# speedinghzl/CCNet

Hardware: NVIDIA H100
Metric: cca_fwd_bwd_pixels_per_s (higher is better)
Workload: dtype f32

## Files before the change

ccnet_b200/csrc/cca_items.cuh:

```cuda
#pragma once

#ifndef __CUDACC__
#define CCA_HD inline
#else
#define CCA_HD __host__ __device__ __forceinline__
#endif

namespace cca {
namespace tc {

constexpr int kMaxTile = 112;
constexpr int kMaxNT = 8;

struct DirGeom {
    int L;
    int NL;
    int nt;
    int tl;
};

struct ItemSpace {
    int B, H, W;
    DirGeom col, row;
    int seg0, seg1, seg2;
    int per_sample, total;
    int nparts;
};

struct Item {
    int col;
    int b, line, iq, ik;
    int q0, lq, k0, lk;
    int j;
};

CCA_HD int tiles_for(int L) { return (L + kMaxTile - 1) / kMaxTile; }

CCA_HD DirGeom make_dir(int L, int NL)
{
    DirGeom g;
    g.L = L; g.NL = NL;
    g.nt = tiles_for(L);
    g.tl = (L + g.nt - 1) / g.nt;
    return g;
}

CCA_HD ItemSpace make_space(int B, int H, int W)
{
    ItemSpace s;
    s.B = B; s.H = H; s.W = W;
    s.col = make_dir(H, W);
    s.row = make_dir(W, H);
    s.seg0 = s.col.NL * s.col.nt;
    s.seg1 = s.col.NL * s.col.nt * (s.col.nt - 1);
    s.seg2 = s.row.NL * s.row.nt * s.row.nt;
    s.per_sample = s.seg0 + s.seg1 + s.seg2;
    s.total = B * s.per_sample;
    s.nparts = s.row.nt + s.col.nt;
    return s;
}

CCA_HD int max_tile(const ItemSpace &s) { return s.col.tl > s.row.tl ? s.col.tl : s.row.tl; }

CCA_HD Item decode_item(const ItemSpace &s, int idx)
{
    Item it;
    it.b = idx / s.per_sample;
    int j = idx - it.b * s.per_sample;
    it.j = j;
    const DirGeom *g;
    if (j < s.seg0) {
        it.col = 1; g = &s.col;
        it.line = j / g->nt; it.iq = j - it.line * g->nt; it.ik = 0;
    } else if (j < s.seg0 + s.seg1) {
        it.col = 1; g = &s.col;
        j -= s.seg0;
        const int per = g->nt - 1;
        const int li = j / per;
        it.ik = 1 + (j - li * per);
        it.line = li / g->nt; it.iq = li - it.line * g->nt;
    } else {
        it.col = 0; g = &s.row;
        j -= s.seg0 + s.seg1;
        const int li = j / g->nt;
        it.ik = j - li * g->nt;
        it.line = li / g->nt; it.iq = li - it.line * g->nt;
    }
    it.q0 = it.iq * g->tl; it.k0 = it.ik * g->tl;
    it.lq = g->L - it.q0 < g->tl ? g->L - it.q0 : g->tl;
    it.lk = g->L - it.k0 < g->tl ? g->L - it.k0 : g->tl;
    return it;
}

CCA_HD Item decode_item_in_sample(const ItemSpace &s, int b, int j) { return decode_item(s, b * s.per_sample + j); }

CCA_HD Item decode_item_lagged(const ItemSpace &s, int idx)
{
    const int np = s.seg0, nc = s.per_sample - s.seg0;
    if (idx < np) return decode_item_in_sample(s, 0, idx);
    const int x = idx - np;
    const int grp = x / s.per_sample, rem = x - grp * s.per_sample;
    if (grp < s.B - 1) {
        if (rem < np) return decode_item_in_sample(s, grp + 1, rem);
        return decode_item_in_sample(s, grp, np + (rem - np));
    }
    (void)nc;
    return decode_item_in_sample(s, s.B - 1, np + rem);
}
CCA_HD Item decode_item_order(const ItemSpace &s, int idx, int lag) { return lag ? decode_item_lagged(s, idx) : decode_item(s, idx); }
CCA_HD bool is_producer(const Item &it) { return it.col && it.ik == 0; }

CCA_HD long item_pixel(const ItemSpace &s, const Item &it, int r)
{
    return it.col ? ((long)it.b * s.H + (it.q0 + r)) * s.W + it.line : ((long)it.b * s.H + it.line) * s.W + (it.q0 + r);
}
CCA_HD int part_index(const ItemSpace &s, const Item &it) { return it.col ? s.row.nt + it.ik : it.ik; }
CCA_HD int qtile_part_index(const ItemSpace &s, const Item &it) { return it.col ? s.row.nt + it.iq : it.iq; }

CCA_HD long zero_share_bytes(long sample_bytes, int per_sample)
{
    const long s = (sample_bytes + per_sample - 1) / per_sample;
    return (s + 127) / 128 * 128;
}

}
}
```

ccnet_b200/csrc/cca_sm90.cuh:

```cuda
#pragma once
#include <cuda.h>
#include <cuda_runtime.h>
#include <stdint.h>

namespace sm90 {

__device__ __forceinline__ uint32_t smem_u32(const void *p) { return (uint32_t)__cvta_generic_to_shared(p); }

__device__ __forceinline__ void mbar_init(uint64_t *bar, uint32_t count)
{
    asm volatile("mbarrier.init.shared::cta.b64 [%0], %1;" ::"r"(smem_u32(bar)), "r"(count));
}
__device__ __forceinline__ void fence_mbar_init() { asm volatile("fence.mbarrier_init.release.cluster;" ::: "memory"); }
__device__ __forceinline__ void mbar_expect_tx(uint64_t *bar, uint32_t bytes)
{
    asm volatile("mbarrier.arrive.expect_tx.shared::cta.b64 _, [%0], %1;" ::"r"(smem_u32(bar)), "r"(bytes) : "memory");
}
__device__ __forceinline__ void mbar_arrive(uint64_t *bar)
{
    asm volatile("mbarrier.arrive.shared::cta.b64 _, [%0];" ::"r"(smem_u32(bar)) : "memory");
}
__device__ __forceinline__ bool mbar_try_wait(uint64_t *bar, uint32_t parity)
{
    uint32_t ok;
    asm volatile(
        "{\n\t.reg .pred p;\n\t"
        "mbarrier.try_wait.parity.shared::cta.b64 p, [%1], %2;\n\t"
        "selp.u32 %0, 1, 0, p;\n\t}"
        : "=r"(ok) : "r"(smem_u32(bar)), "r"(parity) : "memory");
    return ok != 0;
}
#ifndef CCA_SPIN_TRAP
#define CCA_SPIN_TRAP 0
#endif
__device__ __forceinline__ void mbar_wait(uint64_t *bar, uint32_t parity)
{
#if CCA_SPIN_TRAP
    uint32_t spins = 0;
    while (!mbar_try_wait(bar, parity)) {
        if (++spins > (1u << 26)) { __trap(); }
    }
#else
    while (!mbar_try_wait(bar, parity)) {}
#endif
}
__device__ __forceinline__ void wait_count(const unsigned int *cnt, unsigned int need)
{
    unsigned int v;
#if CCA_SPIN_TRAP
    unsigned int spins = 0;
#endif
    for (;;) {
        asm volatile("ld.acquire.gpu.global.u32 %0, [%1];" : "=r"(v) : "l"(cnt) : "memory");
        if (v >= need) return;
        __nanosleep(64);
#if CCA_SPIN_TRAP
        if (++spins > (1u << 24)) __trap();
#endif
    }
}
__device__ __forceinline__ void pdl_launch_dependents() { asm volatile("griddepcontrol.launch_dependents;" ::: "memory"); }
__device__ __forceinline__ void pdl_wait() { asm volatile("griddepcontrol.wait;" ::: "memory"); }

template <int N> __device__ __forceinline__ void setmaxnreg_dec() { asm volatile("setmaxnreg.dec.sync.aligned.u32 %0;" ::"n"(N)); }
template <int N> __device__ __forceinline__ void setmaxnreg_inc() { asm volatile("setmaxnreg.inc.sync.aligned.u32 %0;" ::"n"(N)); }

__device__ __forceinline__ void fence_proxy_async() { asm volatile("fence.proxy.async.shared::cta;" ::: "memory"); }

__device__ __forceinline__ void prefetch_tmap(const CUtensorMap *m)
{
    asm volatile("prefetch.tensormap [%0];" ::"l"(reinterpret_cast<uint64_t>(m)) : "memory");
}
__device__ __forceinline__ void tma_load_4d(void *dst, const CUtensorMap *m, uint64_t *bar, int c0, int c1, int c2, int c3)
{
    asm volatile(
        "cp.async.bulk.tensor.4d.shared::cluster.global.mbarrier::complete_tx::bytes [%0], [%1, {%3, %4, %5, %6}], [%2];"
        ::"r"(smem_u32(dst)), "l"(reinterpret_cast<uint64_t>(m)), "r"(smem_u32(bar)), "r"(c0), "r"(c1), "r"(c2), "r"(c3)
        : "memory");
}
__device__ __forceinline__ uint64_t l2_policy_evict_first()
{
    uint64_t pol;
    asm volatile("createpolicy.fractional.L2::evict_first.b64 %0, 1.0;" : "=l"(pol));
    return pol;
}
__device__ __forceinline__ uint64_t l2_policy_evict_last()
{
    uint64_t pol;
    asm volatile("createpolicy.fractional.L2::evict_last.b64 %0, 1.0;" : "=l"(pol));
    return pol;
}
__device__ __forceinline__ void tma_load_4d(void *dst, const CUtensorMap *m, uint64_t *bar, int c0, int c1, int c2, int c3, uint64_t pol)
{
    asm volatile(
        "cp.async.bulk.tensor.4d.shared::cluster.global.mbarrier::complete_tx::bytes.L2::cache_hint [%0], [%1, {%3, %4, %5, %6}], [%2], %7;"
        ::"r"(smem_u32(dst)), "l"(reinterpret_cast<uint64_t>(m)), "r"(smem_u32(bar)), "r"(c0), "r"(c1), "r"(c2), "r"(c3), "l"(pol)
        : "memory");
}
__device__ __forceinline__ void tma_store_4d(const CUtensorMap *m, const void *src, int c0, int c1, int c2, int c3)
{
    asm volatile("cp.async.bulk.tensor.4d.global.shared::cta.bulk_group [%0, {%2, %3, %4, %5}], [%1];"
                 ::"l"(reinterpret_cast<uint64_t>(m)), "r"(smem_u32(src)), "r"(c0), "r"(c1), "r"(c2), "r"(c3) : "memory");
}
__device__ __forceinline__ void tma_store_4d(const CUtensorMap *m, const void *src, int c0, int c1, int c2, int c3, uint64_t pol)
{
    asm volatile("cp.async.bulk.tensor.4d.global.shared::cta.bulk_group.L2::cache_hint [%0, {%2, %3, %4, %5}], [%1], %6;"
                 ::"l"(reinterpret_cast<uint64_t>(m)), "r"(smem_u32(src)), "r"(c0), "r"(c1), "r"(c2), "r"(c3), "l"(pol) : "memory");
}
__device__ __forceinline__ void tma_reduce_add_4d(const CUtensorMap *m, const void *src, int c0, int c1, int c2, int c3)
{
    asm volatile("cp.reduce.async.bulk.tensor.4d.global.shared::cta.add.tile.bulk_group [%0, {%2, %3, %4, %5}], [%1];"
                 ::"l"(reinterpret_cast<uint64_t>(m)), "r"(smem_u32(src)), "r"(c0), "r"(c1), "r"(c2), "r"(c3) : "memory");
}
__device__ __forceinline__ void tma_reduce_add_4d(const CUtensorMap *m, const void *src, int c0, int c1, int c2, int c3, uint64_t pol)
{
    asm volatile("cp.reduce.async.bulk.tensor.4d.global.shared::cta.add.tile.bulk_group.L2::cache_hint [%0, {%2, %3, %4, %5}], [%1], %6;"
                 ::"l"(reinterpret_cast<uint64_t>(m)), "r"(smem_u32(src)), "r"(c0), "r"(c1), "r"(c2), "r"(c3), "l"(pol) : "memory");
}
__device__ __forceinline__ void bulk_commit() { asm volatile("cp.async.bulk.commit_group;" ::: "memory"); }
template <int N> __device__ __forceinline__ void bulk_wait() { asm volatile("cp.async.bulk.wait_group %0;" ::"n"(N) : "memory"); }
template <int N> __device__ __forceinline__ void bulk_wait_read() { asm volatile("cp.async.bulk.wait_group.read %0;" ::"n"(N) : "memory"); }
__device__ __forceinline__ void fence_proxy_async_global() { asm volatile("fence.proxy.async.global;" ::: "memory"); }
__device__ __forceinline__ void publish_count(unsigned int *cnt)
{
    fence_proxy_async_global();
    __threadfence();
    atomicAdd(cnt, 1u);
}

constexpr uint32_t kSw128 = 1;
__device__ __forceinline__ uint64_t smem_desc(uint32_t smem_addr, uint32_t lbo_bytes, uint32_t sbo_bytes, uint32_t layout_type = 0)
{
    uint64_t d = 0;
    d |= (uint64_t)((smem_addr >> 4) & 0x3FFF);
    d |= (uint64_t)((lbo_bytes >> 4) & 0x3FFF) << 16;
    d |= (uint64_t)((sbo_bytes >> 4) & 0x3FFF) << 32;
    d |= (uint64_t)(layout_type & 3) << 62;
    return d;
}
__device__ __forceinline__ void wg_fence() { asm volatile("wgmma.fence.sync.aligned;" ::: "memory"); }
__device__ __forceinline__ void wg_commit() { asm volatile("wgmma.commit_group.sync.aligned;" ::: "memory"); }
template <int N> __device__ __forceinline__ void wg_wait() { asm volatile("wgmma.wait_group.sync.aligned %0;" ::"n"(N) : "memory"); }
template <int R> __device__ __forceinline__ void wg_acc_fence(float *d)
{
#pragma unroll
    for (int i = 0; i < R; ++i) asm volatile("" : "+f"(d[i])::"memory");
}

#define CCA_WGMMA_SS_N64(AB, TA, TB) asm volatile("{\n.reg .pred p;\nsetp.ne.b32 p, %34, 0;\n" \
    "wgmma.mma_async.sync.aligned.m64n64k16.f32." AB " {%0, %1, %2, %3, %4, %5, %6, %7, %8, %9, %10, %11, %12, %13, %14, %15, %16, %17, %18, %19, %20, %21, %22, %23, %24, %25, %26, %27, %28, %29, %30, %31}, %32, %33, p, 1, 1, " #TA ", " #TB ";\n}" \
    : "+f"(d[0]), "+f"(d[1]), "+f"(d[2]), "+f"(d[3]), "+f"(d[4]), "+f"(d[5]), "+f"(d[6]), "+f"(d[7]), "+f"(d[8]), "+f"(d[9]), "+f"(d[10]), "+f"(d[11]), "+f"(d[12]), "+f"(d[13]), "+f"(d[14]), "+f"(d[15]), "+f"(d[16]), "+f"(d[17]), "+f"(d[18]), "+f"(d[19]), "+f"(d[20]), "+f"(d[21]), "+f"(d[22]), "+f"(d[23]), "+f"(d[24]), "+f"(d[25]), "+f"(d[26]), "+f"(d[27]), "+f"(d[28]), "+f"(d[29]), "+f"(d[30]), "+f"(d[31]) : "l"(a), "l"(b), "r"(scale_d))
#define CCA_WGMMA_SS_N80(AB, TA, TB) asm volatile("{\n.reg .pred p;\nsetp.ne.b32 p, %42, 0;\n" \
    "wgmma.mma_async.sync.aligned.m64n80k16.f32." AB " {%0, %1, %2, %3, %4, %5, %6, %7, %8, %9, %10, %11, %12, %13, %14, %15, %16, %17, %18, %19, %20, %21, %22, %23, %24, %25, %26, %27, %28, %29, %30, %31, %32, %33, %34, %35, %36, %37, %38, %39}, %40, %41, p, 1, 1, " #TA ", " #TB ";\n}" \
    : "+f"(d[0]), "+f"(d[1]), "+f"(d[2]), "+f"(d[3]), "+f"(d[4]), "+f"(d[5]), "+f"(d[6]), "+f"(d[7]), "+f"(d[8]), "+f"(d[9]), "+f"(d[10]), "+f"(d[11]), "+f"(d[12]), "+f"(d[13]), "+f"(d[14]), "+f"(d[15]), "+f"(d[16]), "+f"(d[17]), "+f"(d[18]), "+f"(d[19]), "+f"(d[20]), "+f"(d[21]), "+f"(d[22]), "+f"(d[23]), "+f"(d[24]), "+f"(d[25]), "+f"(d[26]), "+f"(d[27]), "+f"(d[28]), "+f"(d[29]), "+f"(d[30]), "+f"(d[31]), "+f"(d[32]), "+f"(d[33]), "+f"(d[34]), "+f"(d[35]), "+f"(d[36]), "+f"(d[37]), "+f"(d[38]), "+f"(d[39]) : "l"(a), "l"(b), "r"(scale_d))
#define CCA_WGMMA_SS_N112(AB, TA, TB) asm volatile("{\n.reg .pred p;\nsetp.ne.b32 p, %58, 0;\n" \
    "wgmma.mma_async.sync.aligned.m64n112k16.f32." AB " {%0, %1, %2, %3, %4, %5, %6, %7, %8, %9, %10, %11, %12, %13, %14, %15, %16, %17, %18, %19, %20, %21, %22, %23, %24, %25, %26, %27, %28, %29, %30, %31, %32, %33, %34, %35, %36, %37, %38, %39, %40, %41, %42, %43, %44, %45, %46, %47, %48, %49, %50, %51, %52, %53, %54, %55}, %56, %57, p, 1, 1, " #TA ", " #TB ";\n}" \
    : "+f"(d[0]), "+f"(d[1]), "+f"(d[2]), "+f"(d[3]), "+f"(d[4]), "+f"(d[5]), "+f"(d[6]), "+f"(d[7]), "+f"(d[8]), "+f"(d[9]), "+f"(d[10]), "+f"(d[11]), "+f"(d[12]), "+f"(d[13]), "+f"(d[14]), "+f"(d[15]), "+f"(d[16]), "+f"(d[17]), "+f"(d[18]), "+f"(d[19]), "+f"(d[20]), "+f"(d[21]), "+f"(d[22]), "+f"(d[23]), "+f"(d[24]), "+f"(d[25]), "+f"(d[26]), "+f"(d[27]), "+f"(d[28]), "+f"(d[29]), "+f"(d[30]), "+f"(d[31]), "+f"(d[32]), "+f"(d[33]), "+f"(d[34]), "+f"(d[35]), "+f"(d[36]), "+f"(d[37]), "+f"(d[38]), "+f"(d[39]), "+f"(d[40]), "+f"(d[41]), "+f"(d[42]), "+f"(d[43]), "+f"(d[44]), "+f"(d[45]), "+f"(d[46]), "+f"(d[47]), "+f"(d[48]), "+f"(d[49]), "+f"(d[50]), "+f"(d[51]), "+f"(d[52]), "+f"(d[53]), "+f"(d[54]), "+f"(d[55]) : "l"(a), "l"(b), "r"(scale_d))
#define CCA_WGMMA_SS_T(OP, AB) \
    if (ta == 0 && tb == 0) OP(AB, 0, 0); \
    else if (ta == 0) OP(AB, 0, 1); \
    else if (tb == 0) OP(AB, 1, 0); \
    else OP(AB, 1, 1)
template <bool F16 = false> __device__ __forceinline__ void wgmma_ss_n64(float *d, uint64_t a, uint64_t b, int scale_d, int ta, int tb)
{
    if constexpr (F16) { CCA_WGMMA_SS_T(CCA_WGMMA_SS_N64, "f16.f16"); }
    else { CCA_WGMMA_SS_T(CCA_WGMMA_SS_N64, "bf16.bf16"); }
}
template <int TA, int TB> __device__ __forceinline__ void wgmma_ss_n32(float *d, uint64_t a, uint64_t b, int scale_d)
{
    asm volatile("{\n.reg .pred p;\nsetp.ne.b32 p, %18, 0;\n"
        "wgmma.mma_async.sync.aligned.m64n32k16.f32.bf16.bf16 {%0, %1, %2, %3, %4, %5, %6, %7, %8, %9, %10, %11, %12, %13, %14, %15}, %16, %17, p, 1, 1, %19, %20;\n}"
        : "+f"(d[0]), "+f"(d[1]), "+f"(d[2]), "+f"(d[3]), "+f"(d[4]), "+f"(d[5]), "+f"(d[6]), "+f"(d[7]), "+f"(d[8]), "+f"(d[9]), "+f"(d[10]), "+f"(d[11]), "+f"(d[12]), "+f"(d[13]), "+f"(d[14]), "+f"(d[15]) : "l"(a), "l"(b), "r"(scale_d), "n"(TA), "n"(TB));
}
template <bool F16 = false> __device__ __forceinline__ void wgmma_ss_n80(float *d, uint64_t a, uint64_t b, int scale_d, int ta, int tb)
{
    if constexpr (F16) { CCA_WGMMA_SS_T(CCA_WGMMA_SS_N80, "f16.f16"); }
    else { CCA_WGMMA_SS_T(CCA_WGMMA_SS_N80, "bf16.bf16"); }
}
template <bool F16 = false> __device__ __forceinline__ void wgmma_ss_n112(float *d, uint64_t a, uint64_t b, int scale_d, int ta, int tb)
{
    if constexpr (F16) { CCA_WGMMA_SS_T(CCA_WGMMA_SS_N112, "f16.f16"); }
    else { CCA_WGMMA_SS_T(CCA_WGMMA_SS_N112, "bf16.bf16"); }
}
#define CCA_WGMMA_RS_N64(AB) asm volatile("{\n.reg .pred p;\nsetp.ne.b32 p, %37, 0;\n" \
    "wgmma.mma_async.sync.aligned.m64n64k16.f32." AB " {%0, %1, %2, %3, %4, %5, %6, %7, %8, %9, %10, %11, %12, %13, %14, %15, %16, %17, %18, %19, %20, %21, %22, %23, %24, %25, %26, %27, %28, %29, %30, %31}, {%32, %33, %34, %35}, %36, p, 1, 1, 1;\n}" \
    : "+f"(d[0]), "+f"(d[1]), "+f"(d[2]), "+f"(d[3]), "+f"(d[4]), "+f"(d[5]), "+f"(d[6]), "+f"(d[7]), "+f"(d[8]), "+f"(d[9]), "+f"(d[10]), "+f"(d[11]), "+f"(d[12]), "+f"(d[13]), "+f"(d[14]), "+f"(d[15]), "+f"(d[16]), "+f"(d[17]), "+f"(d[18]), "+f"(d[19]), "+f"(d[20]), "+f"(d[21]), "+f"(d[22]), "+f"(d[23]), "+f"(d[24]), "+f"(d[25]), "+f"(d[26]), "+f"(d[27]), "+f"(d[28]), "+f"(d[29]), "+f"(d[30]), "+f"(d[31]) : "r"(a[0]), "r"(a[1]), "r"(a[2]), "r"(a[3]), "l"(b), "r"(scale_d))
template <bool F16 = false> __device__ __forceinline__ void wgmma_rs_n64_tb(float *d, const uint32_t *a, uint64_t b, int scale_d)
{
    if constexpr (F16) CCA_WGMMA_RS_N64("f16.f16");
    else CCA_WGMMA_RS_N64("bf16.bf16");
}

template <int N, bool F16 = false> __device__ __forceinline__ void wgmma_ss(float *d, uint64_t a, uint64_t b, int scale_d, int ta, int tb)
{
    static_assert(N == 64 || N == 80 || N == 112, "wgmma width");
    if constexpr (N == 64) wgmma_ss_n64<F16>(d, a, b, scale_d, ta, tb);
    else if constexpr (N == 80) wgmma_ss_n80<F16>(d, a, b, scale_d, ta, tb);
    else wgmma_ss_n112<F16>(d, a, b, scale_d, ta, tb);
}

}
```

ccnet_b200/csrc/cca_tc_bwd.cuh:

```cuda
#pragma once
#include "cca_items.cuh"
#include "cca_tc_common.cuh"

namespace cca {
namespace tc {

template <int LK, typename E, bool PL = false>
cudaError_t launch_bwd(const void *dout, const void *q, const void *k, const void *v, const void *out, const float *lse, float *delta,
                       unsigned int *counters, void *dq, void *dk, void *dv, Dims d, int delta_mode, cudaStream_t st,
                       const char **why);

struct BwdParams {
    ItemSpace sp;
    int C, Cq;
    long npix;
    const float *lse;
    float *delta;
    unsigned int *ddone;
    int delta_mode;
    int out_mode;
    unsigned int *cdone;
    int lag;
    int hints;
};

template <int LK, typename E> struct BwdSmem {
    using T = Tiles<LK, E>;
    static constexpr int kCh = T::H16 ? kNC : kNC / 2;
    static constexpr int kRSlot = T::kTile;
    static constexpr int off_qk = 0;
    static constexpr int off_p = off_qk + 2 * T::kSlot;
    static constexpr int off_ld = (off_p + T::kP + (16 - LK / 8) * T::kPlane + 1023) / 1024 * 1024;
    static constexpr int kTail = (128 - LK) * 128 + 256;
    static constexpr int kDsum = 1024;
    static constexpr int kBudget = 232448;
    static constexpr int kNLd = (kBudget - off_ld - kTail - kDsum) / (kRSlot + 16);
    static constexpr int off_tail = off_ld + kNLd * kRSlot;
    static constexpr int off_dsum = off_tail + kTail;
    static constexpr int off_bar = off_dsum + kDsum;
    static constexpr int kBytes = off_bar + 8 * 2 * kNLd;
    static_assert(kNLd >= 8, "ring depth: chunk n - 1's dO (staged dV) up to chunk n + 1's O");
    static_assert(off_p % 1024 == 0 && T::kP >= T::kSlot, "dK staging in the P / dS planes");
    static_assert(kBytes <= kBudget, "shared memory budget");
};

__device__ __forceinline__ bool calc_delta(const BwdParams &p, const Item &it) { return p.delta_mode == 0 || (it.col && it.ik == 0); }

template <int LK, typename E, bool PL = false>
__global__ void __launch_bounds__(kThreads, 1)
cca_tc_bwd_kernel(const __grid_constant__ CUtensorMap mqc, const __grid_constant__ CUtensorMap mqr,
                  const __grid_constant__ CUtensorMap mkc, const __grid_constant__ CUtensorMap mkr,
                  const __grid_constant__ CUtensorMap mvc, const __grid_constant__ CUtensorMap mvr,
                  const __grid_constant__ CUtensorMap mdoc, const __grid_constant__ CUtensorMap mdor,
                  const __grid_constant__ CUtensorMap moc, const __grid_constant__ CUtensorMap mor,
                  const __grid_constant__ CUtensorMap mdqc, const __grid_constant__ CUtensorMap mdqr,
                  const __grid_constant__ CUtensorMap mdkc, const __grid_constant__ CUtensorMap mdkr,
                  const __grid_constant__ CUtensorMap mdvc, const __grid_constant__ CUtensorMap mdvr, BwdParams p)
{
    using T = Tiles<LK, E>;
    using S = BwdSmem<LK, E>;
    constexpr bool H16 = kH16<E>, F16 = kF16<E>;
    constexpr int TERMS = H16 ? 1 : 3;
    constexpr int kNLd = S::kNLd;
    constexpr int kCh = S::kCh;
    constexpr int KP = LK / 16;
    constexpr int kQKBoxes = H16 ? 1 : 2;
    constexpr uint32_t LOP = T::kPP * T::kPlane;
    extern __shared__ __align__(1024) uint8_t smem[];
    uint64_t *bars = reinterpret_cast<uint64_t *>(smem + S::off_bar);
    uint64_t *full = bars, *empty = bars + kNLd;
    float *dsum = reinterpret_cast<float *>(smem + S::off_dsum);
    const int tid = threadIdx.x, warp = tid >> 5, lane = tid & 31;
    const int NCH = p.C / kCh;
    const int KQ = p.Cq / 16;
    const int nk = p.sp.total > (int)blockIdx.x ? (p.sp.total - (int)blockIdx.x + (int)gridDim.x - 1) / (int)gridDim.x : 0;
    auto item_of = [&](int k) { return decode_item_order(p.sp, (int)blockIdx.x + k * (int)gridDim.x, p.lag); };

    if (tid == 0) {
        for (int i = 0; i < kNLd; ++i) { mbar_init(&full[i], 1); mbar_init(&empty[i], 1); }
        fence_mbar_init();
        prefetch_tmap(&mqc); prefetch_tmap(&mqr); prefetch_tmap(&mkc); prefetch_tmap(&mkr); prefetch_tmap(&mvc); prefetch_tmap(&mvr);
        prefetch_tmap(&mdoc); prefetch_tmap(&mdor); prefetch_tmap(&moc); prefetch_tmap(&mor);
        prefetch_tmap(&mdqc); prefetch_tmap(&mdqr); prefetch_tmap(&mdkc); prefetch_tmap(&mdkr); prefetch_tmap(&mdvc); prefetch_tmap(&mdvr);
    }
    __syncthreads();

    if (tid < 128) {
        setmaxnreg_dec<kProducerRegs>();
        if (warp == 0 && lane == 0) {
            const uint64_t pol_keep = l2_policy_evict_last(), pol_stream = l2_policy_evict_first();
            uint32_t g = 0;
            auto ring = [&](const CUtensorMap *m, int c0, const Item &it, int start, bool last_use) {
                const int slot = g % kNLd;
                mbar_wait(&empty[slot], ((g / kNLd) & 1) ^ 1);
                mbar_expect_tx(&full[slot], S::kRSlot);
                uint8_t *dst = smem + S::off_ld + slot * S::kRSlot;
                const int cw = it.col ? it.line : start, ch = it.col ? start : it.line;
                if (p.hints == 1) {
                    const uint64_t pol = (is_producer(it) && !last_use) ? pol_keep : pol_stream;
                    tma_load_4d(dst, m, &full[slot], c0, cw, ch, it.b, pol);
                } else {
                    tma_load_4d(dst, m, &full[slot], c0, cw, ch, it.b);
                }
                ++g;
            };
            for (int k = 0; k < nk; ++k) {
                const Item it = item_of(k);
                const bool calc = calc_delta(p, it);
                for (int bx = 0; bx < kQKBoxes; ++bx) ring(it.col ? &mqc : &mqr, 32 * bx, it, it.q0, false);
                for (int bx = 0; bx < kQKBoxes; ++bx) ring(it.col ? &mkc : &mkr, 32 * bx, it, it.k0, false);
                for (int n = 0; n < NCH; ++n) {
                    ring(it.col ? &mvc : &mvr, n * kCh, it, it.k0, false);
                    ring(it.col ? &mdoc : &mdor, n * kCh, it, it.q0, false);
                    if (calc) ring(it.col ? &moc : &mor, n * kCh, it, it.q0, p.delta_mode == 1);
                }
            }
        }
    } else {
        setmaxnreg_inc<kConsumerRegs>();
        const int t = tid - 128, wg = t >> 7, wq = (t >> 5) & 3;
        const int rbase = 64 * wg + 16 * wq + (lane >> 2);
        const int cq = 2 * (lane & 3);
        const uint32_t qb = smem_u32(smem + S::off_qk), kb = qb + T::kSlot, ld_base = smem_u32(smem + S::off_ld);
        const uint32_t pb = smem_u32(smem + S::off_p);
        uint8_t *pgen = smem + S::off_p;
        const uint64_t pol_keep = l2_policy_evict_last(), pol_stream = l2_policy_evict_first();
        auto stage = [&](const float *acc, int nc, uint8_t *tile) {
#pragma unroll
            for (int h = 0; h < 2; ++h) {
                const int r = rbase + 8 * h;
                if (r >= LK) continue;
                uint8_t *row = tile + r * 128;
#pragma unroll
                for (int j = 0; j < 8; ++j) {
                    if (8 * j >= nc) break;
                    const int c = 8 * j + cq;
                    const int bx = H16 ? 0 : c >> 5, byte = H16 ? 2 * c : 4 * (c & 31);
                    uint8_t *dst = row + bx * T::kTile + ((((byte >> 4) ^ r) & 7) << 4) + (byte & 15);
                    if constexpr (H16) *reinterpret_cast<uint32_t *>(dst) = pack2<F16>(acc[4 * j + 2 * h], acc[4 * j + 2 * h + 1]);
                    else *reinterpret_cast<float2 *>(dst) = make_float2(acc[4 * j + 2 * h], acc[4 * j + 2 * h + 1]);
                }
            }
        };
        auto put = [&](const CUtensorMap *m, const uint8_t *tile, int boxes, int c0, int px0, const Item &it, bool prod, int part) {
            const int cw = it.col ? it.line : px0, ch = it.col ? px0 : it.line;
            const int ob = PL ? part * p.sp.B + it.b : it.b;
            for (int bx = 0; bx < boxes; ++bx) {
                const uint8_t *src = tile + bx * T::kTile;
                if (p.hints == 1) {
                    if (prod) tma_store_4d(m, src, c0 + 32 * bx, cw, ch, ob, pol_keep);
                    else tma_reduce_add_4d(m, src, c0 + 32 * bx, cw, ch, ob, pol_stream);
                } else {
                    if (prod) tma_store_4d(m, src, c0 + 32 * bx, cw, ch, ob);
                    else tma_reduce_add_4d(m, src, c0 + 32 * bx, cw, ch, ob);
                }
            }
            bulk_commit();
        };
        const int qboxes = H16 ? 1 : (p.Cq > 32 ? 2 : 1);
        pdl_wait();
        uint32_t g = 0;
        int pending = -1;
        int unpublished = -1;
        for (int k = 0; k < nk; ++k) {
            const Item it = item_of(k);
            const bool calc = calc_delta(p, it);
            const bool prod = PL || (p.out_mode == 1 && is_producer(it));
            long qpix[2];
            bool qok[2];
            float nlse[2];
            int self[2];
#pragma unroll
            for (int h = 0; h < 2; ++h) {
                const int r = rbase + 8 * h;
                qok[h] = r < it.lq;
                qpix[h] = item_pixel(p.sp, it, qok[h] ? r : 0);
                nlse[h] = qok[h] ? -p.lse[qpix[h]] * kLog2e : 0.f;
                self[h] = it.col ? it.q0 + r - it.k0 : -1;
            }
            {
                const uint8_t *src[2 * kQKBoxes];
#pragma unroll
                for (int i = 0; i < 2 * kQKBoxes; ++i) {
                    const uint32_t gi = g + i;
                    mbar_wait(&full[gi % kNLd], (gi / kNLd) & 1);
                    src[i] = smem + S::off_ld + (gi % kNLd) * S::kRSlot;
                }
                if constexpr (H16) {
                    constexpr int kV = T::kTile / 16, kPer = (kV + kConsumers - 1) / kConsumers;
                    uint4 v[2][kPer];
#pragma unroll
                    for (int i = 0; i < 2; ++i)
#pragma unroll
                        for (int j = 0; j < kPer; ++j)
                            if (t + kConsumers * j < kV) v[i][j] = reinterpret_cast<const uint4 *>(src[i])[t + kConsumers * j];
                    consumers_sync();
#pragma unroll
                    for (int i = 0; i < 2; ++i)
#pragma unroll
                        for (int j = 0; j < kPer; ++j)
                            if (t + kConsumers * j < kV) reinterpret_cast<uint4 *>(smem + S::off_qk + i * T::kSlot)[t + kConsumers * j] = v[i][j];
                    fence_proxy_async();
                    consumers_sync();
                } else {
                    convert_slot<LK, E, 4>(smem + S::off_qk, t, nullptr, src);
                }
                if (t == 0)
                    for (int i = 0; i < 2 * kQKBoxes; ++i) mbar_arrive(&empty[(g + i) % kNLd]);
                g += 2 * kQKBoxes;
            }
            {
                float acc[LK / 2];
                wg_fence();
                for (int ks = 0; ks < KQ; ++ks) {
                    wgmma_ss<LK, F16>(acc, desc_kmaj<LK, E>(qb, 64 * wg, ks, false), desc_kmaj<LK, E>(kb, 0, ks, false), ks > 0, 0, 0);
                    if constexpr (TERMS == 3) {
                        wgmma_ss<LK, F16>(acc, desc_kmaj<LK, E>(qb, 64 * wg, ks, false), desc_kmaj<LK, E>(kb, 0, ks, true), 1, 0, 0);
                        wgmma_ss<LK, F16>(acc, desc_kmaj<LK, E>(qb, 64 * wg, ks, true), desc_kmaj<LK, E>(kb, 0, ks, false), 1, 0, 0);
                    }
                }
                wg_commit();
                wg_wait<0>();
                wg_acc_fence<LK / 2>(acc);
                if (t == 0) {
                    if (unpublished >= 0) {
                        bulk_wait<0>();
                        publish_count(p.cdone + unpublished);
                        unpublished = -1;
                    } else {
                        bulk_wait_read<0>();
                    }
                }
                consumers_sync();
#pragma unroll
                for (int j = 0; j < LK / 8; ++j)
#pragma unroll
                    for (int h = 0; h < 2; ++h) {
                        const int r = rbase + 8 * h, c = 8 * j + cq;
                        const bool ok0 = qok[h] && c < it.lk && c != self[h];
                        const bool ok1 = qok[h] && c + 1 < it.lk && c + 1 != self[h];
                        const float p0 = ok0 ? exp2f(fmaf(acc[4 * j + 2 * h], kLog2e, nlse[h])) : 0.f;
                        const float p1 = ok1 ? exp2f(fmaf(acc[4 * j + 2 * h + 1], kLog2e, nlse[h])) : 0.f;
                        if (r < LK) {
                            uint8_t *d = pgen + j * T::kPlane + r * 16 + cq * 2;
                            if constexpr (H16) {
                                *reinterpret_cast<uint32_t *>(d) = pack2<F16>(p0, p1);
                            } else {
                                uint32_t hi, lo;
                                split2(p0, p1, hi, lo);
                                *reinterpret_cast<uint32_t *>(d) = hi;
                                *reinterpret_cast<uint32_t *>(d + LOP) = lo;
                            }
                        }
                    }
            }
            fence_proxy_async();
            consumers_sync();
            float dp[LK / 2];
            float o[kCh / 2];
            float dacc = 0.f;
            const uint32_t per = calc ? 3 : 2;
            auto rslot = [&](uint32_t gi) { return gi % kNLd; };
            auto convert_chunk = [&](int n) {
                const uint32_t gv = g + per * n, gd = gv + 1, go = gv + 2;
                mbar_wait(&full[rslot(gv)], (gv / kNLd) & 1);
                mbar_wait(&full[rslot(gd)], (gd / kNLd) & 1);
                if (calc) mbar_wait(&full[rslot(go)], (go / kNLd) & 1);
                uint8_t *vs = smem + S::off_ld + rslot(gv) * S::kRSlot, *ds = smem + S::off_ld + rslot(gd) * S::kRSlot;
                const uint8_t *os = smem + S::off_ld + rslot(go) * S::kRSlot;
                if constexpr (H16) {
                    if (calc) {
                        dacc += convert_slot<LK, E, 1>(ds, t, os);
                        consumers_sync();
                        if (t == 0) mbar_arrive(&empty[rslot(go)]);
                    }
                } else {
                    const int r = t & 127, hq = t >> 7;
                    const int rr = r < LK ? r : LK - 1, sw = rr & 7;
                    float4 raw[2][4];
#pragma unroll
                    for (int j = 0; j < 4; ++j) {
                        raw[0][j] = *reinterpret_cast<const float4 *>(vs + rr * 128 + (((hq * 4 + j) ^ sw) * 16));
                        raw[1][j] = *reinterpret_cast<const float4 *>(ds + rr * 128 + (((hq * 4 + j) ^ sw) * 16));
                    }
                    if (calc) {
                        float acc = 0.f;
#pragma unroll
                        for (int j = 0; j < 4; ++j) {
                            const float4 o = *reinterpret_cast<const float4 *>(os + rr * 128 + (((hq * 4 + j) ^ sw) * 16));
                            const float4 x = raw[1][j];
                            acc += x.x * o.x + x.y * o.y + x.z * o.z + x.w * o.w;
                        }
                        dacc += r < LK ? acc : 0.f;
                    }
                    named_bar_sync(kBarConvert, kConsumers);
                    if (calc && t == 0) mbar_arrive(&empty[rslot(go)]);
                    if (r < LK) {
#pragma unroll
                        for (int b = 0; b < 2; ++b) {
                            uint8_t *d = (b ? ds : vs) + r * 16 + hq * 2 * T::kPStride;
#pragma unroll
                            for (int j = 0; j < 2; ++j) {
                                const float4 a = raw[b][2 * j], c = raw[b][2 * j + 1];
                                const float v[8] = {a.x, a.y, a.z, a.w, c.x, c.y, c.z, c.w};
                                uint4 hi, lo;
                                split8(v, hi, lo);
                                *reinterpret_cast<uint4 *>(d + j * T::kPStride) = hi;
                                *reinterpret_cast<uint4 *>(d + j * T::kPStride + T::kLoOff) = lo;
                            }
                        }
                    }
                    fence_proxy_async();
                }
            };
            auto issue_dp = [&](int n) {
                const uint32_t gv = g + per * n, gd = gv + 1;
                const uint32_t vb = ld_base + rslot(gv) * S::kRSlot, db = ld_base + rslot(gd) * S::kRSlot;
                wg_fence();
#pragma unroll
                for (int ks = 0; ks < kCh / 16; ++ks) {
                    wgmma_ss<LK, F16>(dp, desc_kmaj<LK, E>(db, 64 * wg, ks, false), desc_kmaj<LK, E>(vb, 0, ks, false), n > 0 || ks > 0, 0, 0);
                    if constexpr (TERMS == 3) {
                        wgmma_ss<LK, F16>(dp, desc_kmaj<LK, E>(db, 64 * wg, ks, false), desc_kmaj<LK, E>(vb, 0, ks, true), 1, 0, 0);
                        wgmma_ss<LK, F16>(dp, desc_kmaj<LK, E>(db, 64 * wg, ks, true), desc_kmaj<LK, E>(vb, 0, ks, false), 1, 0, 0);
                    }
                }
                wg_commit();
            };
            auto issue_dv = [&](int n) {
                const uint32_t db = ld_base + rslot(g + per * n + 1) * S::kRSlot;
                wg_fence();
#pragma unroll
                for (int ks = 0; ks < KP; ++ks) {
                    const uint32_t pa = pb + 8 * wg * T::kPlane + ks * 256;
                    if constexpr (H16) {
                        wgmma_ss_n64<F16>(o, smem_desc(pa, 128, T::kPlane), desc_mnmaj<LK, E>(db, ks, false), ks > 0, 1, 1);
                    } else {
                        wgmma_ss_n32<1, 1>(o, smem_desc(pa, 128, T::kPlane), desc_mnmaj<LK, E>(db, ks, false), ks > 0);
                        wgmma_ss_n32<1, 1>(o, smem_desc(pa, 128, T::kPlane), desc_mnmaj<LK, E>(db, ks, true), 1);
                        wgmma_ss_n32<1, 1>(o, smem_desc(pa + LOP, 128, T::kPlane), desc_mnmaj<LK, E>(db, ks, false), 1);
                    }
                }
                wg_commit();
            };
            auto release = [&]() {
                if (t == 0 && pending >= 0) {
                    bulk_wait_read<0>();
                    mbar_arrive(&empty[pending]);
                    pending = -1;
                }
            };
            convert_chunk(0);
            if constexpr (!H16) consumers_sync();
            issue_dp(0);
            issue_dv(0);
            for (int n = 0; n < NCH; ++n) {
                if (n + 1 < NCH) convert_chunk(n + 1);
                release();
                wg_wait<0>();
                wg_acc_fence<kCh / 2>(o);
                if (n == 0 && !prod) {
                    if (p.out_mode == 1) wait_count(p.cdone + it.b, (unsigned)p.sp.seg0);
                    if (t == 0) fence_proxy_async_global();
                }
                consumers_sync();
                if (t == 0) mbar_arrive(&empty[rslot(g + per * n)]);
                if (n + 1 < NCH) issue_dp(n + 1);
                uint8_t *ds = smem + S::off_ld + rslot(g + per * n + 1) * S::kRSlot;
                stage(o, kCh, ds);
                fence_proxy_async();
                consumers_sync();
                if (t == 0) {
                    put(it.col ? &mdvc : &mdvr, ds, 1, n * kCh, it.k0, it, prod, qtile_part_index(p.sp, it));
                    pending = (int)rslot(g + per * n + 1);
                }
                if (n + 1 < NCH) issue_dv(n + 1);
            }
            wg_wait<0>();
            wg_acc_fence<LK / 2>(dp);
            g += per * NCH;
            float dl[2] = {0.f, 0.f};
            if (calc) {
                dsum[(t >> 7) * 128 + (t & 127)] = dacc;
                consumers_sync();
#pragma unroll
                for (int h = 0; h < 2; ++h) {
                    const int r = rbase + 8 * h;
                    dl[h] = dsum[r] + dsum[128 + r];
                    if (qok[h] && is_producer(it) && (lane & 3) == 0) p.delta[qpix[h]] = dl[h];
                }
                if (p.delta_mode == 1) {
                    __threadfence();
                    consumers_sync();
                    if (t == 0) atomicAdd(p.ddone + it.b, 1u);
                }
            } else {
                wait_count(p.ddone + it.b, (unsigned)p.sp.seg0);
#pragma unroll
                for (int h = 0; h < 2; ++h) dl[h] = qok[h] ? __ldcg(p.delta + qpix[h]) : 0.f;
            }
            consumers_sync();
#pragma unroll
            for (int j = 0; j < LK / 8; ++j)
#pragma unroll
                for (int h = 0; h < 2; ++h) {
                    const int r = rbase + 8 * h;
                    if (r < LK) {
                        uint8_t *d = pgen + j * T::kPlane + r * 16 + cq * 2;
                        const uint32_t hw = *reinterpret_cast<const uint32_t *>(d);
                        const uint32_t lw = H16 ? 0u : *reinterpret_cast<const uint32_t *>(d + LOP);
                        const float p0 = lo2<F16>(hw) + lo2<F16>(lw), p1 = hi2<F16>(hw) + hi2<F16>(lw);
                        const float s0 = qok[h] ? p0 * (dp[4 * j + 2 * h] - dl[h]) : 0.f;
                        const float s1 = qok[h] ? p1 * (dp[4 * j + 2 * h + 1] - dl[h]) : 0.f;
                        if constexpr (H16) {
                            *reinterpret_cast<uint32_t *>(d) = pack2<F16>(s0, s1);
                        } else {
                            uint32_t hi, lo;
                            split2(s0, s1, hi, lo);
                            *reinterpret_cast<uint32_t *>(d) = hi;
                            *reinterpret_cast<uint32_t *>(d + LOP) = lo;
                        }
                    }
                }
            fence_proxy_async();
            consumers_sync();
            {
                float aq[32], ak[32];
                wg_fence();
#pragma unroll
                for (int ks = 0; ks < KP; ++ks) {
                    const uint32_t a = pb + 64 * wg * 16 + ks * 2 * T::kPlane;
                    wgmma_ss_n64<F16>(aq, smem_desc(a, T::kPlane, 128), desc_mnmaj<LK, E>(kb, ks, false), ks > 0, 0, 1);
                    if constexpr (TERMS == 3) {
                        wgmma_ss_n64<F16>(aq, smem_desc(a, T::kPlane, 128), desc_mnmaj<LK, E>(kb, ks, true), 1, 0, 1);
                        wgmma_ss_n64<F16>(aq, smem_desc(a + LOP, T::kPlane, 128), desc_mnmaj<LK, E>(kb, ks, false), 1, 0, 1);
                    }
                }
                wg_commit();
                wg_wait<0>();
                wg_acc_fence<32>(aq);
                consumers_sync();
                stage(aq, 64, smem + S::off_qk + T::kSlot);
                fence_proxy_async();
                consumers_sync();
                if (t == 0) put(it.col ? &mdqc : &mdqr, smem + S::off_qk + T::kSlot, qboxes, 0, it.q0, it, prod, part_index(p.sp, it));
                wg_fence();
#pragma unroll
                for (int ks = 0; ks < KP; ++ks) {
                    const uint32_t at = pb + 8 * wg * T::kPlane + ks * 256;
                    wgmma_ss_n64<F16>(ak, smem_desc(at, 128, T::kPlane), desc_mnmaj<LK, E>(qb, ks, false), ks > 0, 1, 1);
                    if constexpr (TERMS == 3) {
                        wgmma_ss_n64<F16>(ak, smem_desc(at, 128, T::kPlane), desc_mnmaj<LK, E>(qb, ks, true), 1, 1, 1);
                        wgmma_ss_n64<F16>(ak, smem_desc(at + LOP, 128, T::kPlane), desc_mnmaj<LK, E>(qb, ks, false), 1, 1, 1);
                    }
                }
                wg_commit();
                wg_wait<0>();
                wg_acc_fence<32>(ak);
                consumers_sync();
                stage(ak, 64, pgen);
                fence_proxy_async();
                consumers_sync();
                if (t == 0) {
                    put(it.col ? &mdkc : &mdkr, pgen, qboxes, 0, it.k0, it, prod, qtile_part_index(p.sp, it));
                    bulk_wait_read<1>();
                    if (pending >= 0) mbar_arrive(&empty[pending]);
                    pending = -1;
                    if (!PL && prod) unpublished = it.b;
                }
            }
        }
        if (t == 0) {
            bulk_wait<0>();
            if (unpublished >= 0) publish_count(p.cdone + unpublished);
        }
    }
}

namespace {
__global__ void __launch_bounds__(256) cca_bwd_prep_kernel(uint4 *dq, uint4 *dk, uint4 *dv, long nq16, long nv16,
                                                           unsigned int *counters, int n_counters)
{
    pdl_launch_dependents();
    const long tid = (long)blockIdx.x * blockDim.x + threadIdx.x, nth = (long)gridDim.x * blockDim.x;
    const uint4 z = make_uint4(0, 0, 0, 0);
    for (long i = tid; i < nq16; i += nth) { dq[i] = z; dk[i] = z; }
    for (long i = tid; i < nv16; i += nth) dv[i] = z;
    for (long i = tid; i < n_counters; i += nth) counters[i] = 0u;
}
}

template <int LK, typename E, bool PL>
cudaError_t launch_bwd(const void *dout, const void *q, const void *k, const void *v, const void *out, const float *lse, float *delta,
                       unsigned int *counters, void *dq, void *dk, void *dv, Dims d, int delta_mode, cudaStream_t st,
                       const char **why)
{
    CUtensorMap m[16];
    const void *base[8] = {q, k, v, dout, out, dq, dk, dv};
    const int ch[8] = {d.Cq, d.Cq, d.C, d.C, d.C, d.Cq, d.Cq, d.C};
    BwdParams p;
    p.sp = make_space(d.B, d.H, d.W);
    for (int t = 0; t < 8; ++t)
        for (int r = 0; r < 2; ++r) {
            const int box = t < 5 ? LK : (r == 0 ? p.sp.col.tl : p.sp.row.tl);
            const int nb = PL && t >= 5 ? p.sp.nparts * d.B : d.B;
            if (!get_map(&m[2 * t + r], base[t], nb, d.H, d.W, ch[t], box, r == 0, kDtype<E>)) {
                if (why) *why = "cuTensorMapEncodeTiled failed";
                return cudaErrorInvalidValue;
            }
        }
    p.C = d.C; p.Cq = d.Cq;
    p.npix = (long)d.B * d.H * d.W;
    p.lse = lse; p.delta = delta;
    p.ddone = counters; p.cdone = counters + d.B;
    p.delta_mode = delta_mode;
    const bool one_tile = p.sp.col.nt == 1 && p.sp.row.nt == 1;
    p.out_mode = one_tile || PL ? 1 : 0;
    p.lag = tc_lag() != 0 ? 1 : 0;
    p.hints = tc_l2_hints();
    const long es = sizeof(E);
    const long nq = p.out_mode == 1 ? 0 : p.npix * d.Cq * es, nv = p.out_mode == 1 ? 0 : p.npix * d.C * es;
    cca_bwd_prep_kernel<<<p.out_mode == 1 ? 1 : sm_count(), 256, 0, st>>>(
        reinterpret_cast<uint4 *>(dq), reinterpret_cast<uint4 *>(dk), reinterpret_cast<uint4 *>(dv), nq / 16, nv / 16, counters, 3 * d.B);
    count_launch();
    cudaError_t e = cudaGetLastError();
    if (e != cudaSuccess) return e;
    auto kern = cca_tc_bwd_kernel<LK, E, PL>;
    e = cudaFuncSetAttribute(kern, cudaFuncAttributeMaxDynamicSharedMemorySize, BwdSmem<LK, E>::kBytes);
    if (e != cudaSuccess) return e;
    const int sms = sm_count();
    const int grid = p.sp.total < sms ? p.sp.total : sms;
    cudaLaunchConfig_t cfg = {};
    cfg.gridDim = dim3(grid); cfg.blockDim = dim3(kThreads); cfg.dynamicSmemBytes = BwdSmem<LK, E>::kBytes; cfg.stream = st;
    cudaLaunchAttribute attr[1];
    attr[0].id = cudaLaunchAttributeProgrammaticStreamSerialization;
    attr[0].val.programmaticStreamSerializationAllowed = 1;
    cfg.attrs = attr;
    cfg.numAttrs = tc_pdl() ? 1 : 0;
    e = cudaLaunchKernelEx(&cfg, kern, m[0], m[1], m[2], m[3], m[4], m[5], m[6], m[7], m[8], m[9], m[10], m[11], m[12], m[13],
                           m[14], m[15], p);
    count_launch();
    return e != cudaSuccess ? e : cudaGetLastError();
}


extern template cudaError_t launch_bwd<80, __half>(const void *, const void *, const void *, const void *, const void *, const float *,
                                                   float *, unsigned int *, void *, void *, void *, Dims, int, cudaStream_t,
                                                   const char **);
extern template cudaError_t launch_bwd<112, __half>(const void *, const void *, const void *, const void *, const void *, const float *,
                                                    float *, unsigned int *, void *, void *, void *, Dims, int, cudaStream_t,
                                                    const char **);
extern template cudaError_t launch_bwd<80, float, true>(const void *, const void *, const void *, const void *, const void *,
                                                        const float *, float *, unsigned int *, void *, void *, void *, Dims, int,
                                                        cudaStream_t, const char **);
extern template cudaError_t launch_bwd<112, float, true>(const void *, const void *, const void *, const void *, const void *,
                                                         const float *, float *, unsigned int *, void *, void *, void *, Dims, int,
                                                         cudaStream_t, const char **);

}
}
```

ccnet_b200/csrc/cca_tc_fwd.cuh:

```cuda

#pragma once
#include "cca_items.cuh"
#include "cca_tc_common.cuh"

namespace cca {
namespace tc {

template <int LK, typename E, bool PL = false>
cudaError_t launch_fwd(const void *q, const void *k, const void *v, void *out, float *lse, const float *parts, unsigned int *cdone,
                       Dims d, cudaStream_t st, const char **why);

struct FwdParams {
    ItemSpace sp;
    int C, Cq;
    long npix;
    const float *parts;
    float *lse;
    unsigned int *cdone;
    int lag;
    int hints;
};

template <int LK, typename E> struct FwdSmem {
    using T = Tiles<LK, E>;
// ... 133 lines not shown
                float lse2 = 0.f;
                if (rok[h]) {
                    float m = -INFINITY;
#pragma unroll
                    for (int i = 0; i < kPre; ++i)
                        if (i < p.sp.nparts) m = fmaxf(m, pv[h][i]);
                    for (int i = kPre; i < p.sp.nparts; ++i) m = fmaxf(m, __ldcg(p.parts + (long)i * p.npix + pix[h]));
                    float sum = 0.f;
#pragma unroll
                    for (int i = 0; i < kPre; ++i)
                        if (i < p.sp.nparts) sum += exp2f(pv[h][i] - m);
                    for (int i = kPre; i < p.sp.nparts; ++i) sum += exp2f(__ldcg(p.parts + (long)i * p.npix + pix[h]) - m);
                    lse2 = m + log2f(sum);
                    if (!it.col && it.ik == 0 && (lane & 3) == 0) p.lse[pix[h]] = lse2 * kLn2;
                }
                nlse[h] = -lse2;
            }
            wg_wait<0>();
            wg_acc_fence<LK / 2>(acc);
            mbar_arrive(qk_empty);
            uint32_t ph[KP][4], pl[KP][4];
#pragma unroll
            for (int j = 0; j < LK / 8; ++j)
#pragma unroll
                for (int h = 0; h < 2; ++h) {
                    const int c = 8 * j + 2 * (lane & 3);
                    const bool ok0 = rok[h] && c < it.lk && c != self[h];
                    const bool ok1 = rok[h] && c + 1 < it.lk && c + 1 != self[h];
                    const float p0 = ok0 ? exp2f(fmaf(acc[4 * j + 2 * h], kLog2e, nlse[h])) : 0.f;
                    const float p1 = ok1 ? exp2f(fmaf(acc[4 * j + 2 * h + 1], kLog2e, nlse[h])) : 0.f;
                    const int reg = (j & 1) * 2 + h;
                    if constexpr (H16) {
                        ph[j / 2][reg] = pack2<F16>(p0, p1);
                        pl[j / 2][reg] = 0u;
                    } else {
                        split2(p0, p1, ph[j / 2][reg], pl[j / 2][reg]);
                    }
                }
            const uint32_t g0 = g;
            g += NCH;
            const CUtensorMap *const mo = it.col ? &moc : &mor;
            const int ow = it.col ? it.line : it.q0, oh = it.col ? it.q0 : it.line;
            auto slot_of = [&](int n) { return (int)((g0 + n) % kNLd); };
            auto prep = [&](int n) {
                mbar_wait(&full[slot_of(n)], ((g0 + n) / kNLd) & 1);
                if constexpr (!H16) convert_slot<LK, E>(smem + S::off_ld + slot_of(n) * T::kSlot, t);
            };
            auto mma = [&](float (&o)[32], int n) {
                const uint32_t vb = ld_base + slot_of(n) * T::kSlot;
                wg_fence();
#pragma unroll
                for (int ks = 0; ks < KP; ++ks) {
                    wgmma_rs_n64_tb<F16>(o, ph[ks], desc_mnmaj<LK, E>(vb, ks, false), ks > 0);
                    if constexpr (TERMS == 3) {
                        wgmma_rs_n64_tb<F16>(o, ph[ks], desc_mnmaj<LK, E>(vb, ks, true), 1);
                        wgmma_rs_n64_tb<F16>(o, pl[ks], desc_mnmaj<LK, E>(vb, ks, false), 1);
                    }
                }
                wg_commit();
            };
            auto write = [&](float (&o)[32], int n) {
                wg_acc_fence<32>(o);
                consumers_sync();
                stage(o, smem + S::off_ld + slot_of(n) * T::kSlot);
                fence_proxy_async();
                consumers_sync();
            };
            auto store = [&](int n) {
                if (t != 0) return;
                if (n == 0 && !prod) fence_proxy_async_global();
                const uint8_t *sl = smem + S::off_ld + slot_of(n) * T::kSlot;
                const int ob = PL ? part_index(p.sp, it) * p.sp.B + it.b : it.b;
#pragma unroll
                for (int bx = 0; bx < (H16 ? 1 : 2); ++bx) {
                    const int c0 = n * kNC + 32 * bx;
                    const uint8_t *src = sl + bx * T::kTile;
                    if (p.hints == 1) {
                        if (prod) tma_store_4d(mo, src, c0, ow, oh, ob, pol_keep);
                        else tma_reduce_add_4d(mo, src, c0, ow, oh, ob, pol_stream);
                    } else {
                        if (prod) tma_store_4d(mo, src, c0, ow, oh, ob);
                        else tma_reduce_add_4d(mo, src, c0, ow, oh, ob);
                    }
                }
                bulk_commit();
                bulk_wait_read<1>();
                if (pending >= 0) mbar_arrive(&empty[pending]);
                pending = slot_of(n);
            };
            auto acquire = [&](int n) {
                if (n == 0 && !prod) wait_count(p.cdone + it.b, (unsigned)p.sp.seg0);
            };
            auto step = [&](float (&oc)[32], float (&op)[32], int n) {
                if (n > 0) write(op, n - 1);
                const bool more = n + 1 < NCH;
                if (more) prep(n + 1);
                wg_wait<0>();
                if (n > 0) {
                    acquire(n - 1);
                    store(n - 1);
                }
                if (more) mma(op, n + 1);
            };
            float o0[32], o1[32];
            prep(0);
            mma(o0, 0);
            for (int n = 0; n < NCH; n += 2) {
                step(o0, o1, n);
                if (n + 1 < NCH) step(o1, o0, n + 1);
            }
            wg_wait<0>();
            if (NCH & 1) write(o0, NCH - 1);
            else write(o1, NCH - 1);
            acquire(NCH - 1);
            store(NCH - 1);
            if constexpr (!PL) {
                if (prod && t == 0) {
                    bulk_wait<0>();
                    mbar_arrive(&empty[pending]);
                    pending = -1;
                    publish_count(p.cdone + it.b);
                }
            }
        }
        if (t == 0) bulk_wait<0>();
    }
}

template <int LK, typename E, bool PL>
cudaError_t launch_fwd(const void *q, const void *k, const void *v, void *out, float *lse, const float *parts, unsigned int *cdone,
                       Dims d, cudaStream_t st, const char **why)
{
    CUtensorMap m[8];
    const void *base[4] = {q, k, v, out};
    const int ch[4] = {d.Cq, d.Cq, d.C, d.C};
    FwdParams p;
    p.sp = make_space(d.B, d.H, d.W);
    for (int t = 0; t < 4; ++t)
        for (int r = 0; r < 2; ++r) {
            const int box = t < 3 ? LK : (r == 0 ? p.sp.col.tl : p.sp.row.tl);
            const int nb = PL && t == 3 ? p.sp.nparts * d.B : d.B;
            if (!get_map(&m[2 * t + r], base[t], nb, d.H, d.W, ch[t], box, r == 0, kDtype<E>)) {
                if (why) *why = "cuTensorMapEncodeTiled failed";
                return cudaErrorInvalidValue;
            }
        }
    p.C = d.C; p.Cq = d.Cq;
    p.npix = (long)d.B * d.H * d.W;
    p.parts = parts; p.lse = lse; p.cdone = cdone;
    p.hints = tc_l2_hints();
    const int sms = sm_count();
    const int grid = p.sp.total < sms ? p.sp.total : sms;
    const int lag = tc_lag();
    p.lag = lag >= 0 ? lag : (d.B >= 4 && 3 * p.sp.per_sample >= 4 * grid ? 0 : 1);
    auto kern = cca_tc_fwd_kernel<LK, E, PL>;
    cudaError_t e = cudaFuncSetAttribute(kern, cudaFuncAttributeMaxDynamicSharedMemorySize, FwdSmem<LK, E>::kBytes);
    if (e != cudaSuccess) return e;
    cudaLaunchConfig_t cfg = {};
    cfg.gridDim = dim3(grid); cfg.blockDim = dim3(kThreads); cfg.dynamicSmemBytes = FwdSmem<LK, E>::kBytes; cfg.stream = st;
    cudaLaunchAttribute attr[1];
    attr[0].id = cudaLaunchAttributeProgrammaticStreamSerialization;
    attr[0].val.programmaticStreamSerializationAllowed = 1;
    cfg.attrs = attr;
    cfg.numAttrs = tc_pdl() ? 1 : 0;
    e = cudaLaunchKernelEx(&cfg, kern, m[0], m[1], m[2], m[3], m[4], m[5], m[6], m[7], p);
    count_launch();
    return e != cudaSuccess ? e : cudaGetLastError();
}


extern template cudaError_t launch_fwd<80, __half>(const void *, const void *, const void *, void *, float *, const float *,
                                                   unsigned int *, Dims, cudaStream_t, const char **);
extern template cudaError_t launch_fwd<112, __half>(const void *, const void *, const void *, void *, float *, const float *,
                                                    unsigned int *, Dims, cudaStream_t, const char **);
extern template cudaError_t launch_fwd<80, float, true>(const void *, const void *, const void *, void *, float *, const float *,
                                                        unsigned int *, Dims, cudaStream_t, const char **);
extern template cudaError_t launch_fwd<112, float, true>(const void *, const void *, const void *, void *, float *, const float *,
                                                         unsigned int *, Dims, cudaStream_t, const char **);

}
}
```

Measured before the change: 39.20 million.

## Publish backward producer progress per chunk group for finer-grained consumer waits

```diff
diff --git a/ccnet_b200/csrc/cca_items.cuh b/ccnet_b200/csrc/cca_items.cuh
--- a/ccnet_b200/csrc/cca_items.cuh
+++ b/ccnet_b200/csrc/cca_items.cuh
@@ -108,7 +108,12 @@
     return decode_item_in_sample(s, s.B - 1, np + rem);
 }
 CCA_HD Item decode_item_order(const ItemSpace &s, int idx, int lag) { return lag ? decode_item_lagged(s, idx) : decode_item(s, idx); }
+CCA_HD int default_lag(const ItemSpace &s, int grid) { return s.B >= 4 && 3 * s.per_sample >= 4 * grid ? 0 : 1; }
 CCA_HD bool is_producer(const Item &it) { return it.col && it.ik == 0; }
+
+constexpr int kBwdGroups = 4;
+CCA_HD int chunk_group(int n, int nch, int groups) { return n * groups / nch; }
+CCA_HD bool group_end(int n, int nch, int groups) { return chunk_group(n + 1, nch, groups) != chunk_group(n, nch, groups); }
 
 CCA_HD long item_pixel(const ItemSpace &s, const Item &it, int r)
 {
diff --git a/ccnet_b200/csrc/cca_sm90.cuh b/ccnet_b200/csrc/cca_sm90.cuh
--- a/ccnet_b200/csrc/cca_sm90.cuh
+++ b/ccnet_b200/csrc/cca_sm90.cuh
@@ -59,6 +59,34 @@
 #endif
     }
 }
+__device__ __forceinline__ unsigned field7(unsigned long long v, int f) { return (unsigned)(v >> (7 * f)) & 127u; }
+__device__ __forceinline__ unsigned int ld_acquire(const unsigned int *p)
+{
+    unsigned int v;
+    asm volatile("ld.acquire.gpu.global.u32 %0, [%1];" : "=r"(v) : "l"(p) : "memory");
+    return v;
+}
+__device__ __forceinline__ unsigned long long ld_acquire(const unsigned long long *p)
+{
+    unsigned long long v;
+    asm volatile("ld.acquire.gpu.global.u64 %0, [%1];" : "=l"(v) : "l"(p) : "memory");
+    return v;
+}
+template <typename U> __device__ __forceinline__ U wait_field(const U *cnt, U seen, int f, unsigned need)
+{
+#if CCA_SPIN_TRAP
+    unsigned int spins = 0;
+#endif
+    while (field7(seen, f) < need) {
+        seen = ld_acquire(cnt);
+        if (field7(seen, f) >= need) break;
+        __nanosleep(64);
+#if CCA_SPIN_TRAP
+        if (++spins > (1u << 24)) __trap();
+#endif
+    }
+    return seen;
+}
 __device__ __forceinline__ void pdl_launch_dependents() { asm volatile("griddepcontrol.launch_dependents;" ::: "memory"); }
 __device__ __forceinline__ void pdl_wait() { asm volatile("griddepcontrol.wait;" ::: "memory"); }
 
@@ -126,6 +154,12 @@
     fence_proxy_async_global();
     __threadfence();
     atomicAdd(cnt, 1u);
+}
+template <typename U> __device__ __forceinline__ void publish_field(U *cnt, int f)
+{
+    fence_proxy_async_global();
+    __threadfence();
+    atomicAdd(cnt, (U)1 << (7 * f));
 }
 
 constexpr uint32_t kSw128 = 1;
diff --git a/ccnet_b200/csrc/cca_tc_bwd.cuh b/ccnet_b200/csrc/cca_tc_bwd.cuh
--- a/ccnet_b200/csrc/cca_tc_bwd.cuh
+++ b/ccnet_b200/csrc/cca_tc_bwd.cuh
@@ -19,7 +19,7 @@
     unsigned int *ddone;
     int delta_mode;
     int out_mode;
-    unsigned int *cdone;
+    unsigned long long *cdone;
     int lag;
     int hints;
 };
@@ -166,6 +166,9 @@
             const Item it = item_of(k);
             const bool calc = calc_delta(p, it);
             const bool prod = PL || (p.out_mode == 1 && is_producer(it));
+            const bool pub = !PL && prod;
+            unsigned long long *const cd = p.cdone + it.b;
+            unsigned long long seen = 0ull;
             long qpix[2];
             bool qok[2];
             float nlse[2];
@@ -225,7 +228,7 @@
                 if (t == 0) {
                     if (unpublished >= 0) {
                         bulk_wait<0>();
-                        publish_count(p.cdone + unpublished);
+                        publish_field(p.cdone + unpublished, kBwdGroups);
                         unpublished = -1;
                     } else {
                         bulk_wait_read<0>();
@@ -343,8 +346,12 @@
                 }
                 wg_commit();
             };
-            auto release = [&]() {
+            auto release = [&](int n) {
                 if (t == 0 && pending >= 0) {
+                    if (pub && n >= 2 && group_end(n - 2, NCH, kBwdGroups)) {
+                        bulk_wait<1>();
+                        publish_field(cd, chunk_group(n - 2, NCH, kBwdGroups));
+                    }
                     bulk_wait_read<0>();
                     mbar_arrive(&empty[pending]);
                     pending = -1;
@@ -356,12 +363,19 @@
             issue_dv(0);
             for (int n = 0; n < NCH; ++n) {
                 if (n + 1 < NCH) convert_chunk(n + 1);
-                release();
+                release(n);
                 wg_wait<0>();
                 wg_acc_fence<kCh / 2>(o);
-                if (n == 0 && !prod) {
-                    if (p.out_mode == 1) wait_count(p.cdone + it.b, (unsigned)p.sp.seg0);
-                    if (t == 0) fence_proxy_async_global();
+                if (!prod && t == 0) {
+                    if (p.out_mode == 1) {
+                        const int f = chunk_group(n, NCH, kBwdGroups);
+                        if (field7(seen, f) < (unsigned)p.sp.seg0) {
+                            seen = wait_field(cd, seen, f, (unsigned)p.sp.seg0);
+                            fence_proxy_async_global();
+                        }
+                    } else if (n == 0) {
+                        fence_proxy_async_global();
+                    }
                 }
                 consumers_sync();
                 if (t == 0) mbar_arrive(&empty[rslot(g + per * n)]);
@@ -398,6 +412,13 @@
                 wait_count(p.ddone + it.b, (unsigned)p.sp.seg0);
 #pragma unroll
                 for (int h = 0; h < 2; ++h) dl[h] = qok[h] ? __ldcg(p.delta + qpix[h]) : 0.f;
+            }
+            if (t == 0 && pub) {
+                bulk_wait<0>();
+                mbar_arrive(&empty[pending]);
+                pending = -1;
+                if (NCH >= 2 && group_end(NCH - 2, NCH, kBwdGroups)) publish_field(cd, chunk_group(NCH - 2, NCH, kBwdGroups));
+                publish_field(cd, chunk_group(NCH - 1, NCH, kBwdGroups));
             }
             consumers_sync();
 #pragma unroll
@@ -439,6 +460,10 @@
                 wg_commit();
                 wg_wait<0>();
                 wg_acc_fence<32>(aq);
+                if (!prod && p.out_mode == 1 && t == 0) {
+                    seen = wait_field(cd, seen, kBwdGroups, (unsigned)p.sp.seg0);
+                    fence_proxy_async_global();
+                }
                 consumers_sync();
                 stage(aq, 64, smem + S::off_qk + T::kSlot);
                 fence_proxy_async();
@@ -466,13 +491,13 @@
                     bulk_wait_read<1>();
                     if (pending >= 0) mbar_arrive(&empty[pending]);
                     pending = -1;
-                    if (!PL && prod) unpublished = it.b;
+                    if (pub) unpublished = it.b;
                 }
             }
         }
         if (t == 0) {
             bulk_wait<0>();
-            if (unpublished >= 0) publish_count(p.cdone + unpublished);
+            if (unpublished >= 0) publish_field(p.cdone + unpublished, kBwdGroups);
         }
     }
 }
@@ -512,11 +537,14 @@
     p.C = d.C; p.Cq = d.Cq;
     p.npix = (long)d.B * d.H * d.W;
     p.lse = lse; p.delta = delta;
-    p.ddone = counters; p.cdone = counters + d.B;
+    p.cdone = reinterpret_cast<unsigned long long *>(counters);
+    p.ddone = counters + 2 * d.B;
     p.delta_mode = delta_mode;
     const bool one_tile = p.sp.col.nt == 1 && p.sp.row.nt == 1;
     p.out_mode = one_tile || PL ? 1 : 0;
-    p.lag = tc_lag() != 0 ? 1 : 0;
+    const int lag = tc_lag();
+    const int sms0 = sm_count();
+    p.lag = lag >= 0 ? lag : default_lag(p.sp, p.sp.total < sms0 ? p.sp.total : sms0);
     p.hints = tc_l2_hints();
     const long es = sizeof(E);
     const long nq = p.out_mode == 1 ? 0 : p.npix * d.Cq * es, nv = p.out_mode == 1 ? 0 : p.npix * d.C * es;
diff --git a/ccnet_b200/csrc/cca_tc_fwd.cuh b/ccnet_b200/csrc/cca_tc_fwd.cuh
--- a/ccnet_b200/csrc/cca_tc_fwd.cuh
+++ b/ccnet_b200/csrc/cca_tc_fwd.cuh
@@ -309,7 +309,7 @@
     const int sms = sm_count();
     const int grid = p.sp.total < sms ? p.sp.total : sms;
     const int lag = tc_lag();
-    p.lag = lag >= 0 ? lag : (d.B >= 4 && 3 * p.sp.per_sample >= 4 * grid ? 0 : 1);
+    p.lag = lag >= 0 ? lag : default_lag(p.sp, grid);
     auto kern = cca_tc_fwd_kernel<LK, E, PL>;
     cudaError_t e = cudaFuncSetAttribute(kern, cudaFuncAttributeMaxDynamicSharedMemorySize, FwdSmem<LK, E>::kBytes);
     if (e != cudaSuccess) return e;
```

Result: faster. 39.64 million (median of 6 runs) (+1.1%).
